# lucidrains/phenaki-pytorch

Measured on AMD Instinct MI355X. Metric: cvivit_encode_frames_per_sec, higher is better.
Workload: dtype bf16; 1 GPU; BASELINE configs[1]: C-ViViT (dim 512, patch 32, tpatch 2, depth 4+4, LFQ 65536) encode video -> token ids, (8,3,17,256,256) f32 per GPU resident in HBM; global_batch=8, parallelism=batch-shard x1, no data-path collective, hip_graph=True

## Files before the change

### include/phenaki_hip.h

```cpp
#ifndef PHENAKI_HIP_H
#define PHENAKI_HIP_H

#ifdef __cplusplus
extern "C" {
#endif

#define PK_OK 0
#define PK_EINVAL (-1)
#define PK_EALIGN (-2)
#define PK_ELAUNCH (-3)

int pk_gemm(int dtype, int a_is_f32, const void* A, int lda, const void* W, int ldw, int M, int N, int K,
            const float* bias, const float* res, int ldr, void* C, int ldc, int out_is_f32, int act,
            const int* a_rows, void* stream);

int pk_gemm_ex(int dtype, int a_is_f32, const void* A, int lda, const void* W, int ldw, int M, int N, int K,
               const float* bias, const float* res, int ldr, void* C, int ldc, int out_is_f32, int act,
               const int* a_rows, int a_nrows, int variant, void* C2, int ldc2, const float* ln_s, const float* ln_t,
               float ln_eps, const int* row_off, const int* col_off, float* stats_out, const float* ln_stats, int dup_rows,
               void* stream);
int pk_gemm_auto_variant(int dtype, int a_is_f32, int M, int N, int K, int lda, int ldw, int a_nrows);

int pk_layernorm(const float* x, int ldx, const float* gamma, const float* beta, float eps, void* out, int ldo,
                 int out_kind, float* out2, int ldo2, void* raw, int ldraw, int M, int D, int grp, int gstride,
// ... 46 lines not shown
int pk_lfq_aux_codebook(const float* Q, int cd, float inv_n, float coef, float* G, float* hc_part, void* stream);
int pk_lfq_aux_grad(const float* proj, const float* GA, const float* GB, int M, int cd, float alpha, float scale, float wen, float wc2,
                    float* dproj, void* stream);
int pk_lfq_aux_finish(const float* ent, const float* commit, int M, const float* hc_part, int cd, float w_e, float gamma, float w_c, float* out,
                      void* stream);

int pk_rmsnorm(const float* x, int ldx, const float* w, float eps, const unsigned char* rowmask, void* out, int ldo, int out_kind,
               int M, int D, void* stream);
int pk_gated_gelu_tanh(const float* h, int ldh, void* out, int ldo, int out_kind, int M, int F, void* stream);

int pk_layernorm_lfq(const float* x, int ldx, const float* gamma, const float* beta, float eps, const float* wp,
                     const float* bp, long long* ids, float* tokens, int ldt, float* proj, int M, int D, int cd,
                     int pb, int pc, void* stream);

int pk_l2norm_rows(const float* x, int ldx, void* out, int ldo, int out_kind, int M, int D, void* stream);

int pk_embed(const long long* ids_prime, int n_prime, const long long* ids, int n, int nb, const float* tok,
             const float* pos, float* out, void* out_t, int S, int D, void* stream);

int pk_cpb_input(const float* w0, const float* b0, float* out, int d0, int d1, int d2, int nd, int D, void* stream);

int pk_attn_pads(int nq, int n_kv, int nnull, int* nq_pad, int* nk_pad);
int pk_attn_prep(int dtype, const float* q, int ldq, const float* kv, int ldkv, const float* null_kv,
                 const float* q_scale, const float* k_scale, float scale, void* Qp, void* Kp, void* Vt,
                 int S, int h, int nq, int n_kv, int nnull, void* stream);

int pk_qkv_project(int dtype, const void* xq, const void* xkv, int ld, const void* wq, const void* wkv, int ldw, int S, int nseq,
                   int h, int K, const float* q_scale, const float* k_scale, float scale, void* Qp, void* Kp, void* Vt,
                   int nq_pad, int nk_pad, const float* q_ln_s, void* stream);

int pk_qkv_attn(int dtype, const void* xq, const void* xkv, int ld, const void* wq, const void* wkv, int ldw, int S, int n, int h, int K,
                const float* q_scale, const float* k_scale, float scale, const float* bias, long bias_hstride, int bias_ld,
                const float* slopes, int causal, void* O, int ldo, const float* q_ln_s, void* stream);

int pk_q_attn_cached(int dtype, const void* xq, int ld, const void* wq, int ldw, int S, int n, int h, int K, const float* q_scale, float scale,
                     const float* q_ln_s, const void* Kp, const void* Vt, int nk_pad, int n_kv, int nnull,
                     const unsigned char* kmask, void* O, int ldo, void* stream);

int pk_attn_fwd(int dtype, const void* Qp, const void* Kp, const void* Vt, const float* bias, long bias_hstride,
                int bias_ld, const unsigned char* kmask, const float* slopes, int causal, void* O, int ldo,
                int out_is_f32, int S, int h, int nq, int n_kv, int nnull, const float* bias_tab, int tab_len,
                const int* pos_code, int code_off, int tab_run4, float score_bound, void* stream);
int pk_attn_fwd_lse(int dtype, const void* Qp, const void* Kp, const void* Vt, const float* bias, long bias_hstride,
                    int bias_ld, const unsigned char* kmask, const float* slopes, int causal, void* O, int ldo,
                    int out_is_f32, int S, int h, int nq, int n_kv, int nnull, float* lse, void* stream);

int pk_attn_small(const float* q, int ldq, const float* kv, int ldkv, const float* q_scale, const float* k_scale,
                  float scale, const float* bias, long bias_hstride, int bias_ld, const unsigned char* kmask,
                  const float* slopes, int causal, void* O, int ldo, int out_kind, int S, int h, int n, void* stream);

int pk_cfg_mix(const float* x, int ldx, int nb, int n_tot, int n_prime, const int* rows, int nrows, float scale,
               int has_null, void* out, int ldo, int out_is_f32, int D, void* stream);

int pk_vocab_ntiles(int V);
int pk_vocab_sample(int dtype, const void* A, int lda, const void* W, int ldw, const float* bias, int M, int V, int D,
                    float temperature, const float* U, const int* rows, unsigned long long seed,
                    const unsigned long long* seed_dev, int need_lse, void* partials, void* stream);
int pk_vocab_sample_philox(int dtype, const void* A, int lda, const void* W, int ldw, const float* bias, int M, int V, int D, float temperature,
                           const int* rows, unsigned long long torch_seed, unsigned long long philox_offset, unsigned int philox_stride,
                           int need_lse, void* partials, void* stream);
int pk_vocab_reduce(const void* partials, int M, int V, const int* rows, const unsigned char* mask, long long* ids,
                    long long* pred, float* scores, int need_lse, void* stream);

int pk_vocab_ce(int dtype, const void* partials, int M, int V, const void* A, int lda, const void* W, int ldw,
                const float* bias, int D, const long long* targets, const int* rows, float* loss, float* lse_out, void* stream);
int pk_ce_grad_slab(int out_bf16, const float* logits, int ldl, const float* lse, const long long* targets, const int* rows,
// ... 77 lines not shown
```

### phenaki_pytorch_amd/_lib.py

```python
import ctypes
import os

import torch

_HERE = os.path.dirname(os.path.abspath(__file__))
LIB_PATH = os.environ.get('PK_LIB_PATH') or os.path.join(_HERE, 'libphenaki_hip.so')

_P = ctypes.c_void_p
_I = ctypes.c_int
_F = ctypes.c_float
_L = ctypes.c_long
_LL = ctypes.c_longlong
_ULL = ctypes.c_ulonglong

SIGNATURES = {
    'pk_gemm': [_I, _I, _P, _I, _P, _I, _I, _I, _I, _P, _P, _I, _P, _I, _I, _I, _P, _P],
    'pk_gemm_ex': [_I, _I, _P, _I, _P, _I, _I, _I, _I, _P, _P, _I, _P, _I, _I, _I, _P, _I, _I, _P, _I, _P, _P, _F, _P, _P, _P, _P, _I, _P],
    'pk_gemm_auto_variant': [_I, _I, _I, _I, _I, _I, _I, _I],
    'pk_layernorm': [_P, _I, _P, _P, _F, _P, _I, _I, _P, _I, _P, _I, _I, _I, _I, _I, _I, _I, _I, _P],
    'pk_rmsnorm': [_P, _I, _P, _F, _P, _P, _I, _I, _I, _I, _P],
    'pk_gated_gelu_tanh': [_P, _I, _P, _I, _I, _I, _I, _P],
    'pk_l2norm_rows': [_P, _I, _P, _I, _I, _I, _I, _P],
    'pk_patchify_ln': [_P, _I, _I, _I, _I, _I, _I, _I, _I, _I, _I, _P, _P, _F, _P, _I, _I, _P],
    'pk_patch_embed': [_P, _I, _I, _I, _I, _I, _I, _I, _I, _F, _I,
                       _P, _I, _P, _P, _P, _I, _I, _I,
                       _P, _I, _P, _P, _P, _I, _I, _I, _I, _P],
    'pk_patch_embed_slices': [_I],
    'pk_patch_embed_splitk': [_P, _I, _I, _I, _I, _I, _I, _I, _I, _I,
                              _P, _I, _P, _P, _I, _I, _I,
                              _P, _I, _P, _P, _I, _I, _I, _P],
    'pk_patch_embed_finish': [_P, _P, _I, _I, _I, _I, _P, _P, _F, _P, _P, _F, _P, _I, _P, _I, _I, _I, _I, _P],
    'pk_patch_embed_finish_groups': [_P, _I, _I, _P, _I, _P, _I, _P],
    'pk_patch_frame_mask': [_P, _LL, _P, _LL, _P, _I, _I, _I, _I, _I, _I, _I, _I, _I, _I, _P],
    'pk_unpatchify': [_P, _I, _P, _I, _I, _I, _I, _I, _I, _I, _I, _I, _I, _P],
    'pk_sqdiff_partials': [_P, _P, _P, _I, _I, _I, _I, _I, _P, _P],
    'pk_peg': [_P, _P, _P, _P, _P, _I, _I, _I, _I, _I, _I, _P],
    'pk_lfq_encode': [_P, _I, _P, _P, _P, _P, _I, _I, _I, _P],
    'pk_lfq_decode': [_P, _P, _P, _P, _I, _I, _I, _P, _I, _I, _I, _I, _P],
    'pk_lfq_aux_parts': [_I],
    'pk_lfq_aux_prep': [_P, _I, _I, _F, _F, _P, _P, _P, _P, _P],
    'pk_lfq_aux_codebook': [_P, _I, _F, _F, _P, _P, _P],
    'pk_lfq_aux_grad': [_P, _P, _P, _I, _I, _F, _F, _F, _F, _P, _P],
    'pk_lfq_aux_finish': [_P, _P, _I, _P, _I, _F, _F, _F, _P, _P],
    'pk_layernorm_lfq': [_P, _I, _P, _P, _F, _P, _P, _P, _P, _I, _P, _I, _I, _I, _I, _I, _P],
    'pk_embed': [_P, _I, _P, _I, _I, _P, _P, _P, _P, _I, _I, _P],
    'pk_cpb_input': [_P, _P, _P, _I, _I, _I, _I, _I, _P],
    'pk_attn_pads': [_I, _I, _I, ctypes.POINTER(_I), ctypes.POINTER(_I)],
    'pk_attn_prep': [_I, _P, _I, _P, _I, _P, _P, _P, _F, _P, _P, _P, _I, _I, _I, _I, _I, _P],
    'pk_qkv_project': [_I, _P, _P, _I, _P, _P, _I, _I, _I, _I, _I, _P, _P, _F, _P, _P, _P, _I, _I, _P, _P],
    'pk_qkv_attn': [_I, _P, _P, _I, _P, _P, _I, _I, _I, _I, _I, _P, _P, _F, _P, _L, _I, _P, _I, _P, _I, _P, _P],
    'pk_q_attn_cached': [_I, _P, _I, _P, _I, _I, _I, _I, _I, _P, _F, _P, _P, _P, _I, _I, _I, _P, _P, _I, _P],
    'pk_attn_fwd': [_I, _P, _P, _P, _P, _L, _I, _P, _P, _I, _P, _I, _I, _I, _I, _I, _I, _I, _P, _I, _P, _I, _I, _F, _P],
    'pk_attn_fwd_lse': [_I, _P, _P, _P, _P, _L, _I, _P, _P, _I, _P, _I, _I, _I, _I, _I, _I, _I, _P, _P],
    'pk_attn_small': [_P, _I, _P, _I, _P, _P, _F, _P, _L, _I, _P, _P, _I, _P, _I, _I, _I, _I, _I, _P],
    'pk_cfg_mix': [_P, _I, _I, _I, _I, _P, _I, _F, _I, _P, _I, _I, _I, _P],
    'pk_vocab_ntiles': [_I],
    'pk_vocab_sample_philox': [_I, _P, _I, _P, _I, _P, _I, _I, _I, _F, _P, _ULL, _ULL, ctypes.c_uint, _I, _P, _P],
    'pk_vocab_sample': [_I, _P, _I, _P, _I, _P, _I, _I, _I, _F, _P, _P, _ULL, _P, _I, _P, _P],
    'pk_vocab_reduce': [_P, _I, _I, _P, _P, _P, _P, _P, _I, _P],
    'pk_vocab_ce': [_I, _P, _I, _I, _P, _I, _P, _I, _P, _I, _P, _P, _P, _P, _P],
    'pk_ce_grad_slab': [_I, _P, _I, _P, _P, _P, _I, _I, _I, _F, _P, _P, _I, _P, _I, _P, _P],
    'pk_topk_mask': [_P, _I, _I, _I, _LL, _P, _P, _P, _P, _P],
    'pk_critic_head': [_P, _I, _P, _P, _I, _I, _I, _I, _I, _F, _P, _F, _ULL, _P, _P, _P],
    'pk_pack': [_P, _LL, _P, _I, _I, _I, _P, _LL, _I, _I, _P],
    'pk_scatter_rows': [_P, _LL, _P, _P, _LL, _I, _I, _P],
    'pk_colsum_parts': [_I],
    'pk_colsum': [_P, _LL, _I, _I, _F, _P, _I, _P, _P],
    'pk_ln_bwd_parts': [_I],
    'pk_layernorm_bwd': [_P, _LL, _P, _P, _LL, _P, _LL, _P, _LL, _P, _P, _F, _I, _I, _P],
    'pk_geglu': [_P, _LL, _I, _P, _LL, _I, _I, _P],
    'pk_geglu_bwd': [_P, _LL, _I, _P, _LL, _P, _LL, _I, _I, _P],
    'pk_leaky_bwd': [_P, _LL, _P, _LL, _P, _LL, _I, _I, _F, _P],
    'pk_scaled_diff': [_P, _P, _F, _P, _P, _LL, _P],
    'pk_sign': [_P, _F, _P, _LL, _P],
    'pk_mul': [_P, _P, _P, _LL, _P],
    'pk_peg_wgrad_parts': [_LL],
    'pk_peg_bwd': [_P, _P, _P, _P, _P, _I, _I, _I, _I, _I, _I, _P],
    'pk_embed_bwd': [_P, _P, _F, _P, _P, _I, _I, _I, _P],
    'pk_bias_gather': [_P, _I, _P, _I, _P, _I, _I, _P],
    'pk_bias_scatter': [_P, _P, _I, _P, _I, _I, _I, _P],
    'pk_sum_batch': [_P, _LL, _I, _P, _LL, _P],
    'pk_sum_batch_multi': [_P, _I, _P],
    'pk_peg_adjoint': [_P, _P, _P, _I, _I, _I, _I, _I, _I, _P],
# ... 278 lines not shown


def attn_prep(dtype, q, kv, null_kv, q_scale, k_scale, scale, Qp, Kp, Vt, S, h, nq, n_kv, nnull):
    rc = load().pk_attn_prep(dtype, ptr(q), q.stride(-2), ptr(kv), kv.stride(-2) if kv is not None else 0, f32p(null_kv, 'null_kv') if nnull else None,
                             f32p(q_scale, 'q_scale'), f32p(k_scale, 'k_scale'), scale, ptr(Qp), ptr(Kp), ptr(Vt), S, h, nq, n_kv, nnull, stream(q))
    _check(rc, 'pk_attn_prep')


def rmsnorm(x, w, M, D, out, eps=1e-6, rowmask=None):
    rc = load().pk_rmsnorm(f32p(x, 'x', rows_ok=True), x.stride(-2), f32p(w, 'T5LayerNorm weight'), eps, ptr(rowmask), ptr(out), out.stride(-2),
                           1 if out.dtype == torch.bfloat16 else 0, M, D, stream(x))
    _check(rc, 'pk_rmsnorm')


def gated_gelu_tanh(h, out, M, F):
    rc = load().pk_gated_gelu_tanh(ptr(h), h.stride(-2), ptr(out), out.stride(-2), 1 if out.dtype == torch.bfloat16 else 0, M, F, stream(h))
    _check(rc, 'pk_gated_gelu_tanh')


def _qkv_dtype(xq):
    if xq.dtype == torch.bfloat16:
        return BF16
    if xq.dtype == torch.float32:
        return BF16X3
    raise RuntimeError(f'fused projection kernels take bf16 (bf16 mode) or f32 (bf16x3 mode) rows, got {xq.dtype}')


def qkv_project(xq, xkv, wq, wkv, S, nseq, h, K, q_scale, k_scale, scale, Qp, Kp, Vt, nq_pad, nk_pad, q_ln_s=None):
    rc = load().pk_qkv_project(_qkv_dtype(xq), ptr(xq), ptr(xkv), xq.stride(-2), ptr(wq), ptr(wkv), wq.stride(0), S, nseq, h, K, f32p(q_scale, 'q_scale'),
                                f32p(k_scale, 'k_scale'), scale, ptr(Qp), ptr(Kp), ptr(Vt), nq_pad, nk_pad, ptr(q_ln_s), stream(xq))
    _check(rc, 'pk_qkv_project')


def qkv_attn(xq, xkv, wq, wkv, S, n, h, K, q_scale, k_scale, scale, O, *, bias=None, slopes=None, causal=False, q_ln_s=None):
    bh, bld = (bias.stride(0), bias.stride(1)) if bias is not None else (0, 0)
    rc = load().pk_qkv_attn(_qkv_dtype(xq), ptr(xq), ptr(xkv), xq.stride(-2), ptr(wq), ptr(wkv), wq.stride(0), S, n, h, K, f32p(q_scale, 'q_scale'),
                            f32p(k_scale, 'k_scale'), scale, f32p(bias, 'attention bias'), bh, bld, f32p(slopes, 'ALiBi slopes'),
                            1 if causal else 0, ptr(O), O.stride(-2), ptr(q_ln_s), stream(xq))
    _check(rc, 'pk_qkv_attn')


def q_attn_cached(xq, wq, S, n, h, K, q_scale, scale, Kp, Vt, nk_pad, n_kv, nnull, O, *, kmask=None, q_ln_s=None):
    rc = load().pk_q_attn_cached(_qkv_dtype(xq), ptr(xq), xq.stride(-2), ptr(wq), wq.stride(0), S, n, h, K, f32p(q_scale, 'q_scale'), scale, ptr(q_ln_s),
                                 ptr(Kp), ptr(Vt), nk_pad, n_kv, nnull, ptr(kmask), ptr(O), O.stride(-2), stream(xq))
    _check(rc, 'pk_q_attn_cached')


def attn_fwd(dtype, Qp, Kp, Vt, O, S, h, nq, n_kv, nnull, *, bias=None, kmask=None, slopes=None, causal=False, bias_table=None,
             score_bound=None, lse=None):
    tab, codes, off = bias_table[:3] if bias_table is not None else (None, None, 0)
    run4 = 1 if (bias_table is not None and len(bias_table) > 5 and bias_table[5]) else 0
    if bias is not None:
        bh, bld = bias.stride(0), bias.stride(1)
    else:
        bh, bld = 0, 0
    if lse is not None:
        assert bias_table is None and score_bound is None
        rc = load().pk_attn_fwd_lse(dtype, ptr(Qp), ptr(Kp), ptr(Vt), ptr(bias), bh, bld, ptr(kmask), f32p(slopes, 'ALiBi slopes'),
                                    1 if causal else 0, ptr(O), O.stride(-2), 1 if O.dtype == torch.float32 else 0, S, h, nq, n_kv, nnull, ptr(lse), stream(O))
        _check(rc, 'pk_attn_fwd_lse')
        return
    rc = load().pk_attn_fwd(dtype, ptr(Qp), ptr(Kp), ptr(Vt), ptr(bias), bh, bld, ptr(kmask), f32p(slopes, 'ALiBi slopes'),
                            1 if causal else 0, ptr(O), O.stride(-2), 1 if O.dtype == torch.float32 else 0,
                            S, h, nq, n_kv, nnull, f32p(tab, 'bias table'), tab.shape[1] if tab is not None else 0, ptr(codes), off, run4,
                            float('nan') if score_bound is None else float(score_bound), stream(O))
    _check(rc, 'pk_attn_fwd')


def attn_small(q, kv, q_scale, k_scale, scale, O, S, h, n, *, bias=None, kmask=None, slopes=None, causal=False):
    bh, bld = (bias.stride(0), bias.stride(1)) if bias is not None else (0, 0)
    rc = load().pk_attn_small(ptr(q), q.stride(-2), ptr(kv), kv.stride(-2), f32p(q_scale, 'q_scale'), f32p(k_scale, 'k_scale'), scale, ptr(bias), bh, bld,
                              ptr(kmask), f32p(slopes, 'ALiBi slopes'), 1 if causal else 0, ptr(O), O.stride(-2),
# ... 383 lines not shown
```

### phenaki_pytorch_amd/csrc/gemm_dma.hpp

```cpp
#pragma once
#include "gemm_core.hpp"

namespace pk {

__device__ __forceinline__ void dot2acc_bf16(float& d, uint32_t a, uint32_t b) {
    asm("v_dot2c_f32_bf16 %0, %1, %2" : "+v"(d) : "v"(a), "v"(b));
}
__device__ __forceinline__ void frag_stats(const Frag<bf16>& f, float& s, float& q, bool want_sq) {
    const uint32_t w0 = f.v[0], w1 = f.v[1], w2 = f.v[2], w3 = f.v[3];
    const uint32_t ones = 0x3f803f80u;
    dot2acc_bf16(s, w0, ones); dot2acc_bf16(s, w1, ones); dot2acc_bf16(s, w2, ones); dot2acc_bf16(s, w3, ones);
    if (want_sq) { dot2acc_bf16(q, w0, w0); dot2acc_bf16(q, w1, w1); dot2acc_bf16(q, w2, w2); dot2acc_bf16(q, w3, w3); }
}
__device__ __forceinline__ void frag_stats(const Frag<float>& f, float& s, float& q, bool want_sq) {
#pragma unroll
    for (int e = 0; e < 4; ++e) {
        s += f.lo[e] + f.hi[e];
        if (want_sq) q = fmaf(f.lo[e], f.lo[e], fmaf(f.hi[e], f.hi[e], q));
    }
}

#ifdef PK_TIMELINE
__device__ unsigned long long pk_tl[8 * 5 * 40];
#define PK_TL(slot) do { if (tl_on && kt < 38) pk_tl[(tl_wg * 40 + kt) * 5 + (slot)] = __builtin_amdgcn_s_memtime(); } while (0)
// ... 137 lines not shown
#pragma unroll
            for (int c = 0; c < CH; ++c) {
                Frag<T> fa[TM], fw[TN];
#pragma unroll
                for (int i = 0; i < TM; ++i) lds_frag_a<T>(fa[i], a, wm * 16 * TM + i * 16 + lr, c, g);
#pragma unroll
                for (int j = 0; j < TN; ++j) lds_frag_w<T>(fw[j], w, wn * 16 * TN + j * 16 + lr, c, g);
#pragma unroll
                for (int i = 0; i < TM; ++i)
#pragma unroll
                    for (int j = 0; j < TN; ++j) acc[i][j] = mma(fw[j], fa[i], acc[i][j]);
                if (STATS) {
#pragma unroll
                    for (int i = 0; i < TM; ++i) frag_stats(fa[i], rsum[i], rsq[i], STATS > 1);
                }
            }
            PK_TL(4);
        }
        if (STATS) {
#pragma unroll
            for (int i = 0; i < TM; ++i) {
                rsum[i] += __shfl_xor(rsum[i], 16, 64);
                rsum[i] += __shfl_xor(rsum[i], 32, 64);
                if (STATS > 1) {
                    rsq[i] += __shfl_xor(rsq[i], 16, 64);
                    rsq[i] += __shfl_xor(rsq[i], 32, 64);
                }
            }
        }
        asm volatile("s_waitcnt lgkmcnt(0)" ::: "memory");
        __builtin_amdgcn_s_barrier();
        return computes;
    }
};

}
```

### phenaki_pytorch_amd/csrc/qkv_attn.hip

```cpp
#include "gemm_dma.hpp"

namespace pk {

struct QkvAttnArgs {
    const void* xq; const void* xkv;
    const void* wq; const void* wkv;
    int ld, ldw;
    int S, n, h, K;
    int spt;
    const float* q_scale; const float* k_scale; float scale;
    const float* bias; long bias_hstride; int bias_ld;
    const float* slopes; int causal;
    void* O; int ldo;
    uint32_t recip;
    const float* q_ln_s;
};

template <typename T> using QaTile = GemmDma<T, 1, 4, 4, 1, 2, 128>;
template <typename T> using QaKvTile = GemmDma<T, 1, 8, 4, 1, 2, 128>;
constexpr int QA_SMEM = QaKvTile<bf16>::SMEM;
static_assert(QaKvTile<bf16x3>::SMEM == QA_SMEM, "the split-bf16 ring has the same bytes");

constexpr int QA_PLANE = 8192;
template <typename T> struct QaImg { static constexpr int PLANES = 1; };
template <> struct QaImg<bf16x3> { static constexpr int PLANES = 2; };
__device__ __forceinline__ void qa_put4(bf16, char* img, int off, f32x4 v) {
    *reinterpret_cast<u32x2*>(img + off) = u32x2{pack_bf2(v[0], v[1]), pack_bf2(v[2], v[3])};
}
__device__ __forceinline__ void qa_put4(bf16x3, char* img, int off, f32x4 v) {
    const uint32_t h0 = pack_bf2(v[0], v[1]), h1 = pack_bf2(v[2], v[3]);
    const float r0 = v[0] - __builtin_bit_cast(float, h0 << 16), r1 = v[1] - __builtin_bit_cast(float, h0 & 0xFFFF0000u);
    const float r2 = v[2] - __builtin_bit_cast(float, h1 << 16), r3 = v[3] - __builtin_bit_cast(float, h1 & 0xFFFF0000u);
    *reinterpret_cast<u32x2*>(img + off) = u32x2{h0, h1};
    *reinterpret_cast<u32x2*>(img + QA_PLANE + off) = u32x2{pack_bf2(r0, r1), pack_bf2(r2, r3)};
}
__device__ __forceinline__ void qa_put1(bf16, char* img, int off, float v) { *reinterpret_cast<u16*>(img + off) = f2bf(v); }
__device__ __forceinline__ void qa_put1(bf16x3, char* img, int off, float v) {
    const u16 h = f2bf(v);
    *reinterpret_cast<u16*>(img + off) = h;
    *reinterpret_cast<u16*>(img + QA_PLANE + off) = f2bf(v - bf2f(h));
}
__device__ __forceinline__ void qa_get(Frag<bf16>& f, const char* img, int off) { f.v = *reinterpret_cast<const u32x4*>(img + off); }
__device__ __forceinline__ void qa_get(Frag<bf16x3>& f, const char* img, int off) {
    f.hi = *reinterpret_cast<const u32x4*>(img + off);
    f.lo = *reinterpret_cast<const u32x4*>(img + QA_PLANE + off);
}

__device__ __forceinline__ int qa_kperm(int f, int i) { return (f >> 1) * 32 + (i >> 2) * 8 + (f & 1) * 4 + (i & 3); }
__device__ __forceinline__ int qa_ksw(int row) { return ((row >> 1) & 1) | (((row >> 3) & 3) << 1); }

template <typename T>
__device__ __forceinline__ void qa_project_q(const GemmOperands& p, int M, int m0, int hh, int K, const float* q_scale, float scale,
                                             const float* q_ln_s, char* smem, char* Qs) {
    const int lane = threadIdx.x & 63, g = lane >> 4, lr = lane & 15;
    const int rq = __builtin_amdgcn_readfirstlane(threadIdx.x >> 6) * 16 + lr;
    f32x4 acc[1][4];
#pragma unroll
    for (int j = 0; j < 4; ++j) acc[0][j] = f32x4{0, 0, 0, 0};
    if (q_ln_s) {
        float rsum[1], rsq[1];
        (void)QaTile<T>::template run_stats<1>(p, M, m0, hh * 64, smem, acc, rsum, rsq);
        const float mean = rsum[0] / (float)K;
#pragma unroll
        for (int j = 0; j < 4; ++j) {
            const f32x4 s4 = *reinterpret_cast<const f32x4*>(q_ln_s + hh * 64 + j * 16 + g * 4);
#pragma unroll
            for (int r = 0; r < 4; ++r) acc[0][j][r] -= mean * s4[r];
        }
    } else {
        (void)QaTile<T>::run(p, M, m0, hh * 64, smem, acc);
    }
    float ss = 0.f;
#pragma unroll
    for (int j = 0; j < 4; ++j)
#pragma unroll
        for (int r = 0; r < 4; ++r) ss += acc[0][j][r] * acc[0][j][r];
    ss += __shfl_xor(ss, 16, 64);
    ss += __shfl_xor(ss, 32, 64);
    const float inv = scale / fmaxf(sqrtf(ss), 1e-12f);
#pragma unroll
    for (int j = 0; j < 4; ++j) {
        const f32x4 sc = *reinterpret_cast<const f32x4*>(q_scale + j * 16 + g * 4);
        f32x4 v = acc[0][j];
#pragma unroll
        for (int r = 0; r < 4; ++r) v[r] *= inv * sc[r];
        const int slot = (2 * j + (g >> 1)) ^ (rq & 7);
        qa_put4(T{}, Qs, rq * 128 + (slot << 4) + (g & 1) * 8, v);
    }
}

template <typename T>
__global__ __launch_bounds__(256) void qkv_attn_kernel(const QkvAttnArgs a) {
    extern __shared__ __attribute__((aligned(16))) char smem[];
    constexpr int NPL = QaImg<T>::PLANES;
    char* Qs = smem;
    char* Ks = smem;
    char* Vts = smem + NPL * QA_PLANE;
    const int R = a.spt * a.n;
    const int tiles = (a.S + a.spt - 1) / a.spt;
    const int xcd = blockIdx.x & 7, idx = blockIdx.x >> 3;
    const int tile = (idx / a.h) * 8 + xcd, hh = idx % a.h;
    if (tile >= tiles) return;
    const int M = a.S * a.n;
    const int m0 = tile * R;
    const int lane = threadIdx.x & 63, g = lane >> 4, lr = lane & 15;
    const int wave = __builtin_amdgcn_readfirstlane(threadIdx.x >> 6);
    const int rq = wave * 16 + lr;

    GemmOperands p;
    p.a_rows = nullptr;
    p.lda = a.ld; p.ldw = a.ldw;
    p.M = M; p.K = a.K;
    p.plain_map = 0; p.krot = 0;
    p.w_gap_from = 0; p.w_gap_rows = 0;

    p.A = a.xq; p.W = a.wq; p.N = a.h * 64;
    qa_project_q<T>(p, M, m0, hh, a.K, a.q_scale, a.scale, a.q_ln_s, smem, Qs);
    Frag<T> fq[2];
    asm volatile("s_waitcnt lgkmcnt(0)" ::: "memory");
#pragma unroll
    for (int c = 0; c < 2; ++c) qa_get(fq[c], Qs, rq * 128 + (((c * 4 + g) ^ (rq & 7)) << 4));
    asm volatile("s_waitcnt lgkmcnt(0)" ::: "memory");
    __builtin_amdgcn_s_barrier();

    {
        f32x4 acc[1][8];
#pragma unroll
        for (int j = 0; j < 8; ++j) acc[0][j] = f32x4{0, 0, 0, 0};
        p.A = a.xkv; p.W = a.wkv; p.N = 2 * a.h * 64;
        p.w_gap_from = 64; p.w_gap_rows = (a.h - 1) * 64;
        (void)QaKvTile<T>::run(p, M, m0, hh * 64, smem, acc);
        float ss = 0.f;
#pragma unroll
        for (int j = 0; j < 4; ++j)
#pragma unroll
            for (int r = 0; r < 4; ++r) ss += acc[0][j][r] * acc[0][j][r];
        ss += __shfl_xor(ss, 16, 64);
        ss += __shfl_xor(ss, 32, 64);
        const float inv = 1.0f / fmaxf(sqrtf(ss), 1e-12f);
#pragma unroll
        for (int j = 0; j < 4; ++j) {
            const f32x4 sc = *reinterpret_cast<const f32x4*>(a.k_scale + j * 16 + g * 4);
            f32x4 v = acc[0][j];
#pragma unroll
            for (int r = 0; r < 4; ++r) v[r] *= inv * sc[r];
            const int slot = (2 * j + (g >> 1)) ^ qa_ksw(rq);
            qa_put4(T{}, Ks, rq * 128 + (slot << 4) + (g & 1) * 8, v);
        }
#pragma unroll
        for (int j = 0; j < 4; ++j)
#pragma unroll
            for (int r = 0; r < 4; ++r) {
                const int d = j * 16 + g * 4 + r;
                qa_put1(T{}, Vts, d * 128 + ((((rq >> 3) ^ (d & 7))) << 4) + (rq & 7) * 2, acc[0][4 + j][r]);
            }
    }
    asm volatile("s_waitcnt lgkmcnt(0)" ::: "memory");
    __builtin_amdgcn_s_barrier();

    f32x4 st[4];
#pragma unroll
    for (int f = 0; f < 4; ++f) st[f] = f32x4{0, 0, 0, 0};
#pragma unroll
    for (int f = 0; f < 4; ++f) {
// ... 179 lines not shown
    mx = fmaxf(mx, __shfl_xor(mx, 32, 64));
    float ls = 0.f;
#pragma unroll
    for (int e = 0; e < 4 * NF; ++e) { pr[e] = __expf(pr[e] - mx); ls += pr[e]; }
    ls += __shfl_xor(ls, 16, 64);
    ls += __shfl_xor(ls, 32, 64);
    f32x4 o[4];
#pragma unroll
    for (int df = 0; df < 4; ++df) o[df] = f32x4{0, 0, 0, 0};
#pragma unroll
    for (int kc = 0; kc < NF / 2; ++kc) {
        Frag<T> fp;
        {
            const float p8[8] = {pr[kc * 8 + 0], pr[kc * 8 + 1], pr[kc * 8 + 2], pr[kc * 8 + 3], pr[kc * 8 + 4], pr[kc * 8 + 5], pr[kc * 8 + 6], pr[kc * 8 + 7]};
            frag_from_f32(fp, p8);
        }
#pragma unroll
        for (int df = 0; df < 4; ++df) {
            const int d = df * 16 + lr;
            Frag<T> fv;
            qa_get(fv, Vts, d * 128 + (((kc * 4 + g) ^ (d & 7)) << 4));
            o[df] = mma(fv, fp, o[df]);
        }
    }
    const float inv = 1.0f / ls;
    T* orow = reinterpret_cast<T*>(a.O) + (size_t)(m0 + rq) * a.ldo + hh * 64;
#pragma unroll
    for (int df = 0; df < 4; ++df) store4(orow + df * 16 + g * 4, o[df] * inv);
}

}
using namespace pk;

extern "C" int pk_qkv_attn(int dtype, const void* xq, const void* xkv, int ld, const void* wq, const void* wkv, int ldw, int S, int n, int h,
                           int K, const float* q_scale, const float* k_scale, float scale, const float* bias, long bias_hstride,
                           int bias_ld, const float* slopes, int causal, void* O, int ldo, const float* q_ln_s, void* stream) {
    if (dtype != 1 && dtype != 2) return PK_EINVAL;
    if (!xq || !xkv || !wq || !wkv || !q_scale || !k_scale || !O || S <= 0 || n <= 0 || n > 64 || h <= 0 || K <= 0) return PK_EINVAL;
    auto mis = [](const void* ptr) { return (reinterpret_cast<uintptr_t>(ptr) & 15) != 0; };
    const int q = dtype == 1 ? 7 : 3, bk = dtype == 1 ? 64 : 32, esz = dtype == 1 ? 2 : 4;
    if ((K & q) || (ld & q) || (ldw & q) || (ldo & 3) || mis(xq) || mis(xkv) || mis(wq) || mis(wkv) || mis(q_scale) || mis(k_scale) ||
        (reinterpret_cast<uintptr_t>(O) & (dtype == 1 ? 7 : 15)) || (bias && mis(bias))) return PK_EALIGN;
    if (ldw < (K + bk - 1) / bk * bk) return PK_EINVAL;
    const long M = (long)S * n;
    if ((size_t)M * ld * esz >= 0xFFFFFFF0ull || (size_t)2 * h * 64 * ldw * esz >= 0xFFFFFFF0ull) return PK_EINVAL;
    QkvAttnArgs a;
    a.xq = xq; a.xkv = xkv; a.wq = wq; a.wkv = wkv; a.ld = ld; a.ldw = ldw;
    a.S = S; a.n = n; a.h = h; a.K = K; a.spt = 64 / n;
    a.q_scale = q_scale; a.k_scale = k_scale; a.scale = scale;
    a.bias = bias; a.bias_hstride = bias_hstride; a.bias_ld = bias_ld;
    a.slopes = slopes; a.causal = causal;
    a.O = O; a.ldo = ldo;
    a.recip = (65536u + (uint32_t)n - 1u) / (uint32_t)n;
    a.q_ln_s = q_ln_s;
    if (q_ln_s && mis(q_ln_s)) return PK_EALIGN;
    const int tiles = (S + a.spt - 1) / a.spt;
    dim3 grid(8 * ((tiles + 7) / 8) * h);
    hipStream_t st = reinterpret_cast<hipStream_t>(stream);
    if (dtype == 1) hipLaunchKernelGGL(qkv_attn_kernel<bf16>, grid, dim3(256), QA_SMEM, st, a);
    else hipLaunchKernelGGL(qkv_attn_kernel<bf16x3>, grid, dim3(256), QA_SMEM, st, a);
    PK_CHECK_LAUNCH();
    return PK_OK;
}

extern "C" int pk_q_attn_cached(int dtype, const void* xq, int ld, const void* wq, int ldw, int S, int n, int h, int K, const float* q_scale,
                                float scale, const float* q_ln_s, const void* Kp, const void* Vt, int nk_pad, int n_kv, int nnull,
                                const unsigned char* kmask, void* O, int ldo, void* stream) {
    if (dtype != 1 && dtype != 2) return PK_EINVAL;
    if (!xq || !wq || !q_scale || !Kp || !Vt || !O || S <= 0 || n <= 0 || (n & 63) || h <= 0 || K <= 0 || n_kv <= 0 || nnull < 0) return PK_EINVAL;
    const int nk = nnull + n_kv;
    if (nk > 64 || nk_pad < nk || nk_pad > 64 || (nk_pad & 31)) return PK_EINVAL;
    auto mis = [](const void* ptr) { return (reinterpret_cast<uintptr_t>(ptr) & 15) != 0; };
    const int q = dtype == 1 ? 7 : 3, bk = dtype == 1 ? 64 : 32, esz = dtype == 1 ? 2 : 4;
    if ((K & q) || (ld & q) || (ldw & q) || (ldo & 3) || mis(xq) || mis(wq) || mis(q_scale) || mis(Kp) || mis(Vt) ||
        (reinterpret_cast<uintptr_t>(O) & (dtype == 1 ? 7 : 15)) || (q_ln_s && mis(q_ln_s))) return PK_EALIGN;
    if (dtype == 2 && ((reinterpret_cast<uintptr_t>(Kp) | reinterpret_cast<uintptr_t>(Vt)) & 127)) return PK_EALIGN;
    if (ldw < (K + bk - 1) / bk * bk) return PK_EINVAL;
    const long M = (long)S * n;
    if ((size_t)M * ld * esz >= 0xFFFFFFF0ull || (size_t)h * 64 * ldw * esz >= 0xFFFFFFF0ull) return PK_EINVAL;
    QAttnCachedArgs a{xq, wq, ld, ldw, S, n, h, K, q_scale, scale, q_ln_s, Kp, Vt, nk_pad, nk, nnull, kmask, n_kv, O, ldo};
    const int tiles = (int)(M / 64);
    dim3 grid(8 * ((tiles + 7) / 8) * h);
    hipStream_t st = reinterpret_cast<hipStream_t>(stream);
    if (dtype == 1) {
        constexpr int lds = QaTile<bf16>::SMEM + 2 * QA_PLANE;
        if (nk_pad > 32) hipLaunchKernelGGL((q_attn_cached_kernel<bf16, true>), grid, dim3(256), lds, st, a);
        else hipLaunchKernelGGL((q_attn_cached_kernel<bf16, false>), grid, dim3(256), lds, st, a);
    } else {
        constexpr int lds = QaTile<bf16x3>::SMEM + 4 * QA_PLANE;
        if (nk_pad > 32) hipLaunchKernelGGL((q_attn_cached_kernel<bf16x3, true>), grid, dim3(256), lds, st, a);
        else hipLaunchKernelGGL((q_attn_cached_kernel<bf16x3, false>), grid, dim3(256), lds, st, a);
    }
    PK_CHECK_LAUNCH();
    return PK_OK;
}
// ... 1 lines not shown
```

Before: 177,200 frames/s.

## Overlap K/V projection prefetch with Q projection tail in fused qkv-attention kernel

```diff
diff --git a/include/phenaki_hip.h b/include/phenaki_hip.h
--- a/include/phenaki_hip.h
+++ b/include/phenaki_hip.h
@@ -102,6 +102,9 @@
 int pk_qkv_attn(int dtype, const void* xq, const void* xkv, int ld, const void* wq, const void* wkv, int ldw, int S, int n, int h, int K,
                 const float* q_scale, const float* k_scale, float scale, const float* bias, long bias_hstride, int bias_ld,
                 const float* slopes, int causal, void* O, int ldo, const float* q_ln_s, void* stream);
+int pk_qkv_attn_ex(int dtype, const void* xq, const void* xkv, int ld, const void* wq, const void* wkv, int ldw, int S, int n, int h, int K,
+                   const float* q_scale, const float* k_scale, float scale, const float* bias, long bias_hstride, int bias_ld,
+                   const float* slopes, int causal, void* O, int ldo, const float* q_ln_s, int sched, void* stream);
 
 int pk_q_attn_cached(int dtype, const void* xq, int ld, const void* wq, int ldw, int S, int n, int h, int K, const float* q_scale, float scale,
                      const float* q_ln_s, const void* Kp, const void* Vt, int nk_pad, int n_kv, int nnull,
diff --git a/phenaki_pytorch_amd/_lib.py b/phenaki_pytorch_amd/_lib.py
--- a/phenaki_pytorch_amd/_lib.py
+++ b/phenaki_pytorch_amd/_lib.py
@@ -49,6 +49,7 @@
     'pk_attn_prep': [_I, _P, _I, _P, _I, _P, _P, _P, _F, _P, _P, _P, _I, _I, _I, _I, _I, _P],
     'pk_qkv_project': [_I, _P, _P, _I, _P, _P, _I, _I, _I, _I, _I, _P, _P, _F, _P, _P, _P, _I, _I, _P, _P],
     'pk_qkv_attn': [_I, _P, _P, _I, _P, _P, _I, _I, _I, _I, _I, _P, _P, _F, _P, _L, _I, _P, _I, _P, _I, _P, _P],
+    'pk_qkv_attn_ex': [_I, _P, _P, _I, _P, _P, _I, _I, _I, _I, _I, _P, _P, _F, _P, _L, _I, _P, _I, _P, _I, _P, _I, _P],
     'pk_q_attn_cached': [_I, _P, _I, _P, _I, _I, _I, _I, _I, _P, _F, _P, _P, _P, _I, _I, _I, _P, _P, _I, _P],
     'pk_attn_fwd': [_I, _P, _P, _P, _P, _L, _I, _P, _P, _I, _P, _I, _I, _I, _I, _I, _I, _I, _P, _I, _P, _I, _I, _F, _P],
     'pk_attn_fwd_lse': [_I, _P, _P, _P, _P, _L, _I, _P, _P, _I, _P, _I, _I, _I, _I, _I, _I, _I, _P, _P],
@@ -393,12 +394,15 @@
     _check(rc, 'pk_qkv_project')
 
 
-def qkv_attn(xq, xkv, wq, wkv, S, n, h, K, q_scale, k_scale, scale, O, *, bias=None, slopes=None, causal=False, q_ln_s=None):
+QKV_ATTN_PIPE = 0 if os.environ.get('PK_QKV_ATTN_PIPE', '1') == '0' else 1
+
+
+def qkv_attn(xq, xkv, wq, wkv, S, n, h, K, q_scale, k_scale, scale, O, *, bias=None, slopes=None, causal=False, q_ln_s=None, sched=None):
     bh, bld = (bias.stride(0), bias.stride(1)) if bias is not None else (0, 0)
-    rc = load().pk_qkv_attn(_qkv_dtype(xq), ptr(xq), ptr(xkv), xq.stride(-2), ptr(wq), ptr(wkv), wq.stride(0), S, n, h, K, f32p(q_scale, 'q_scale'),
-                            f32p(k_scale, 'k_scale'), scale, f32p(bias, 'attention bias'), bh, bld, f32p(slopes, 'ALiBi slopes'),
-                            1 if causal else 0, ptr(O), O.stride(-2), ptr(q_ln_s), stream(xq))
-    _check(rc, 'pk_qkv_attn')
+    rc = load().pk_qkv_attn_ex(_qkv_dtype(xq), ptr(xq), ptr(xkv), xq.stride(-2), ptr(wq), ptr(wkv), wq.stride(0), S, n, h, K, f32p(q_scale, 'q_scale'),
+                               f32p(k_scale, 'k_scale'), scale, f32p(bias, 'attention bias'), bh, bld, f32p(slopes, 'ALiBi slopes'),
+                               1 if causal else 0, ptr(O), O.stride(-2), ptr(q_ln_s), QKV_ATTN_PIPE if sched is None else sched, stream(xq))
+    _check(rc, 'pk_qkv_attn_ex')
 
 
 def q_attn_cached(xq, wq, S, n, h, K, q_scale, scale, Kp, Vt, nk_pad, n_kv, nnull, O, *, kmask=None, q_ln_s=None):
diff --git a/phenaki_pytorch_amd/csrc/gemm_dma.hpp b/phenaki_pytorch_amd/csrc/gemm_dma.hpp
--- a/phenaki_pytorch_amd/csrc/gemm_dma.hpp
+++ b/phenaki_pytorch_amd/csrc/gemm_dma.hpp
@@ -193,6 +193,130 @@
         __builtin_amdgcn_s_barrier();
         return computes;
     }
+
+    struct Feed {
+        __amdgpu_buffer_rsrc_t rsA, rsW;
+        uint32_t offA[IA], offW[IW], bytesA;
+        int wave, nt, rot;
+        bool slot_in_tail;
+
+        __device__ __forceinline__ Feed(const GemmOperands& p, int a_nrows, int m0, int n0, int wave_) : wave(wave_) {
+            constexpr int SZ = (int)sizeof(T);
+            const int lane = threadIdx.x & 63;
+            bytesA = (uint32_t)a_nrows * (uint32_t)p.lda * SZ;
+            const uint32_t bytesW = (uint32_t)p.N * (uint32_t)p.ldw * SZ;
+            rsA = __builtin_amdgcn_make_buffer_rsrc(const_cast<void*>(p.A), 0, bytesA, 0x00020000);
+            rsW = __builtin_amdgcn_make_buffer_rsrc(const_cast<void*>(p.W), 0, bytesW, 0x00020000);
+            const int lrow = lane / SLOTS, lslot = lane % SLOTS;
+            const int srcslot = lslot ^ (lrow & 7);
+#pragma unroll
+            for (int i = 0; i < IA; ++i) {
+                const int row = (wave * IA + i) * RPI + lrow;
+                int gm = m0 + row;
+                const bool ok = gm < p.M;
+                if (ok && p.a_rows) gm = p.a_rows[gm];
+                offA[i] = ok ? (uint32_t)gm * (uint32_t)p.lda * SZ + srcslot * 16 : bytesA;
+            }
+#pragma unroll
+            for (int i = 0; i < IW; ++i) {
+                const int row = (wave * IW + i) * RPI + lrow;
+                const int gn = n0 + row + ((p.w_gap_from > 0 && row >= p.w_gap_from) ? p.w_gap_rows : 0);
+                offW[i] = gn < p.N ? (uint32_t)gn * (uint32_t)p.ldw * SZ + srcslot * 16 : bytesW;
+            }
+            nt = (p.K + BK - 1) / BK;
+            rot = (p.krot && nt > 1) ? (int)(((blockIdx.x >> 3) + blockIdx.y) % (unsigned)nt) : 0;
+            const int ktail_bytes = (p.K * SZ) % ROWB;
+            slot_in_tail = ktail_bytes == 0 || srcslot * 16 < ktail_bytes;
+        }
+
+        __device__ __forceinline__ void issue(int kt, char* base) const {
+            int kk = kt + rot;
+            if (kk >= nt) kk -= nt;
+            const int koff = kk * ROWB;
+            const bool cut = kk == nt - 1 && !slot_in_tail;
+#pragma unroll
+            for (int i = 0; i < IA; ++i)
+                __builtin_amdgcn_raw_ptr_buffer_load_lds(rsA, (lds_ptr)(base + (wave * IA + i) * 1024), 16, cut ? bytesA : offA[i], koff, 0, 0);
+#pragma unroll
+            for (int i = 0; i < IW; ++i)
+                __builtin_amdgcn_raw_ptr_buffer_load_lds(rsW, (lds_ptr)(base + BM * ROWB + (wave * IW + i) * 1024), 16, offW[i], koff, 0, 0);
+        }
+    };
+
+    template <int STATS>
+    static __device__ __forceinline__ void mma_tile(const char* a, int wm, int wn, int lr, int g, f32x4 (&acc)[TM][TN], float (&rsum)[TM],
+                                                    float (&rsq)[TM]) {
+        const char* w = a + BM * ROWB;
+#pragma unroll
+        for (int c = 0; c < CH; ++c) {
+            Frag<T> fa[TM], fw[TN];
+#pragma unroll
+            for (int i = 0; i < TM; ++i) lds_frag_a<T>(fa[i], a, wm * 16 * TM + i * 16 + lr, c, g);
+#pragma unroll
+            for (int j = 0; j < TN; ++j) lds_frag_w<T>(fw[j], w, wn * 16 * TN + j * 16 + lr, c, g);
+#pragma unroll
+            for (int i = 0; i < TM; ++i)
+#pragma unroll
+                for (int j = 0; j < TN; ++j) acc[i][j] = mma(fw[j], fa[i], acc[i][j]);
+            if (STATS) {
+#pragma unroll
+                for (int i = 0; i < TM; ++i) frag_stats(fa[i], rsum[i], rsq[i], STATS > 1);
+            }
+        }
+    }
+
+    template <int STATS>
+    static __device__ __forceinline__ void fold_stats(float (&rsum)[TM], float (&rsq)[TM]) {
+        if (STATS) {
+#pragma unroll
+            for (int i = 0; i < TM; ++i) {
+                rsum[i] += __shfl_xor(rsum[i], 16, 64);
+                rsum[i] += __shfl_xor(rsum[i], 32, 64);
+                if (STATS > 1) {
+                    rsq[i] += __shfl_xor(rsq[i], 16, 64);
+                    rsq[i] += __shfl_xor(rsq[i], 32, 64);
+                }
+            }
+        }
+    }
+
+    template <int STATS, bool ISSUED0, bool CLOSE, typename Seam>
+    static __device__ __forceinline__ void chain(const Feed& feed, char* st0, char* st1, f32x4 (&acc)[TM][TN], float (&rsum)[TM],
+                                                 float (&rsq)[TM], Seam seam) {
+        static_assert(STAGES == 2 && PW == 0, "chained passes: 2-stage ring, no producer waves");
+        const int lane = threadIdx.x & 63, g = lane >> 4, lr = lane & 15;
+        const int cw = feed.wave, wm = cw / WN, wn = cw % WN;
+        const int nt = feed.nt;
+        if (STATS) {
+#pragma unroll
+            for (int i = 0; i < TM; ++i) { rsum[i] = 0.f; rsq[i] = 0.f; }
+        }
+        if (!ISSUED0) feed.issue(0, st0);
+        for (int kt = 0; kt < nt - 1; ++kt) {
+            wait_tiles<0>();
+            __builtin_amdgcn_s_barrier();
+            feed.issue(kt + 1, (kt + 1) & 1 ? st1 : st0);
+            mma_tile<STATS>(kt & 1 ? st1 : st0, wm, wn, lr, g, acc, rsum, rsq);
+        }
+        wait_tiles<0>();
+        __builtin_amdgcn_s_barrier();
+        seam();
+        mma_tile<STATS>((nt - 1) & 1 ? st1 : st0, wm, wn, lr, g, acc, rsum, rsq);
+        fold_stats<STATS>(rsum, rsq);
+        if (CLOSE) {
+            asm volatile("s_waitcnt lgkmcnt(0)" ::: "memory");
+            __builtin_amdgcn_s_barrier();
+        }
+    }
+    template <int STATS, typename Seam>
+    static __device__ __forceinline__ void run_lead(const Feed& feed, char* st0, char* st1, f32x4 (&acc)[TM][TN], float (&rsum)[TM],
+                                                    float (&rsq)[TM], Seam seam) {
+        chain<STATS, false, false>(feed, st0, st1, acc, rsum, rsq, seam);
+    }
+    static __device__ __forceinline__ void run_issued(const Feed& feed, char* st0, char* st1, f32x4 (&acc)[TM][TN]) {
+        float dummy[TM];
+        chain<0, true, true>(feed, st0, st1, acc, dummy, dummy, [] {});
+    }
 };
 
 }
diff --git a/phenaki_pytorch_amd/csrc/qkv_attn.hip b/phenaki_pytorch_amd/csrc/qkv_attn.hip
--- a/phenaki_pytorch_amd/csrc/qkv_attn.hip
+++ b/phenaki_pytorch_amd/csrc/qkv_attn.hip
@@ -50,6 +50,38 @@
 __device__ __forceinline__ int qa_ksw(int row) { return ((row >> 1) & 1) | (((row >> 3) & 3) << 1); }
 
 template <typename T>
+__device__ __forceinline__ void qa_finish_q(f32x4 (&acc)[1][4], bool has_ln, float rsum, int K, const f32x4 (&ln4)[4], const f32x4 (&qs4)[4],
+                                            float scale, char* Qs, int rq, int g) {
+    if (has_ln) {
+        const float mean = rsum / (float)K;
+#pragma unroll
+        for (int j = 0; j < 4; ++j)
+#pragma unroll
+            for (int r = 0; r < 4; ++r) acc[0][j][r] -= mean * ln4[j][r];
+    }
+    float ss = 0.f;
+#pragma unroll
+    for (int j = 0; j < 4; ++j)
+#pragma unroll
+        for (int r = 0; r < 4; ++r) ss += acc[0][j][r] * acc[0][j][r];
+    ss += __shfl_xor(ss, 16, 64);
+    ss += __shfl_xor(ss, 32, 64);
+    const float inv = scale / fmaxf(sqrtf(ss), 1e-12f);
+#pragma unroll
+    for (int j = 0; j < 4; ++j) {
+        f32x4 v = acc[0][j];
+#pragma unroll
+        for (int r = 0; r < 4; ++r) v[r] *= inv * qs4[j][r];
+        const int slot = (2 * j + (g >> 1)) ^ (rq & 7);
+        qa_put4(T{}, Qs, rq * 128 + (slot << 4) + (g & 1) * 8, v);
+    }
+}
+__device__ __forceinline__ void qa_load_cols(f32x4 (&v)[4], const float* base, int g) {
+#pragma unroll
+    for (int j = 0; j < 4; ++j) v[j] = *reinterpret_cast<const f32x4*>(base + j * 16 + g * 4);
+}
+
+template <typename T>
 __device__ __forceinline__ void qa_project_q(const GemmOperands& p, int M, int m0, int hh, int K, const float* q_scale, float scale,
                                              const float* q_ln_s, char* smem, char* Qs) {
     const int lane = threadIdx.x & 63, g = lane >> 4, lr = lane & 15;
@@ -57,40 +89,21 @@
     f32x4 acc[1][4];
 #pragma unroll
     for (int j = 0; j < 4; ++j) acc[0][j] = f32x4{0, 0, 0, 0};
+    float rsum[1] = {0.f}, rsq[1];
+    f32x4 ln4[4], qs4[4];
     if (q_ln_s) {
-        float rsum[1], rsq[1];
         (void)QaTile<T>::template run_stats<1>(p, M, m0, hh * 64, smem, acc, rsum, rsq);
-        const float mean = rsum[0] / (float)K;
-#pragma unroll
-        for (int j = 0; j < 4; ++j) {
-            const f32x4 s4 = *reinterpret_cast<const f32x4*>(q_ln_s + hh * 64 + j * 16 + g * 4);
-#pragma unroll
-            for (int r = 0; r < 4; ++r) acc[0][j][r] -= mean * s4[r];
-        }
+        qa_load_cols(ln4, q_ln_s + hh * 64, g);
     } else {
         (void)QaTile<T>::run(p, M, m0, hh * 64, smem, acc);
     }
-    float ss = 0.f;
-#pragma unroll
-    for (int j = 0; j < 4; ++j)
-#pragma unroll
-        for (int r = 0; r < 4; ++r) ss += acc[0][j][r] * acc[0][j][r];
-    ss += __shfl_xor(ss, 16, 64);
-    ss += __shfl_xor(ss, 32, 64);
-    const float inv = scale / fmaxf(sqrtf(ss), 1e-12f);
-#pragma unroll
-    for (int j = 0; j < 4; ++j) {
-        const f32x4 sc = *reinterpret_cast<const f32x4*>(q_scale + j * 16 + g * 4);
-        f32x4 v = acc[0][j];
-#pragma unroll
-        for (int r = 0; r < 4; ++r) v[r] *= inv * sc[r];
-        const int slot = (2 * j + (g >> 1)) ^ (rq & 7);
-        qa_put4(T{}, Qs, rq * 128 + (slot << 4) + (g & 1) * 8, v);
-    }
-}
-
-template <typename T>
+    qa_load_cols(qs4, q_scale, g);
+    qa_finish_q<T>(acc, q_ln_s != nullptr, rsum[0], K, ln4, qs4, scale, Qs, rq, g);
+}
+
+template <typename T, bool PIPE>
 __global__ __launch_bounds__(256) void qkv_attn_kernel(const QkvAttnArgs a) {
+    static_assert(!PIPE || QaImg<T>::PLANES == 1, "the seam-free schedule stages ONE 8 KB q^ plane beside the k|v stage being filled");
     extern __shared__ __attribute__((aligned(16))) char smem[];
     constexpr int NPL = QaImg<T>::PLANES;
     char* Qs = smem;
@@ -114,22 +127,55 @@
     p.plain_map = 0; p.krot = 0;
     p.w_gap_from = 0; p.w_gap_rows = 0;
 
-    p.A = a.xq; p.W = a.wq; p.N = a.h * 64;
-    qa_project_q<T>(p, M, m0, hh, a.K, a.q_scale, a.scale, a.q_ln_s, smem, Qs);
     Frag<T> fq[2];
-    asm volatile("s_waitcnt lgkmcnt(0)" ::: "memory");
-#pragma unroll
-    for (int c = 0; c < 2; ++c) qa_get(fq[c], Qs, rq * 128 + (((c * 4 + g) ^ (rq & 7)) << 4));
-    asm volatile("s_waitcnt lgkmcnt(0)" ::: "memory");
-    __builtin_amdgcn_s_barrier();
-
-    {
-        f32x4 acc[1][8];
-#pragma unroll
-        for (int j = 0; j < 8; ++j) acc[0][j] = f32x4{0, 0, 0, 0};
+    f32x4 acc[1][8];
+#pragma unroll
+    for (int j = 0; j < 8; ++j) acc[0][j] = f32x4{0, 0, 0, 0};
+    if constexpr (PIPE) {
+        using QT = QaTile<T>;
+        using KT = QaKvTile<T>;
+        const int nt = (a.K + QT::BK - 1) / QT::BK;
+        const int s0 = nt & 1;
+        char* const kv0 = smem + s0 * KT::STAGE_BYTES;
+        char* const kv1 = smem + (s0 ^ 1) * KT::STAGE_BYTES;
+        Qs = smem + (s0 ? 2 : 3) * QA_PLANE;
+        p.A = a.xq; p.W = a.wq; p.N = a.h * 64;
+        const typename QT::Feed feed_q(p, M, m0, hh * 64, wave);
+        p.A = a.xkv; p.W = a.wkv; p.N = 2 * a.h * 64;
+        p.w_gap_from = 64; p.w_gap_rows = (a.h - 1) * 64;
+        const typename KT::Feed feed_kv(p, M, m0, hh * 64, wave);
+        f32x4 qacc[1][4];
+#pragma unroll
+        for (int j = 0; j < 4; ++j) qacc[0][j] = f32x4{0, 0, 0, 0};
+        float rsum[1] = {0.f}, rsq[1];
+        f32x4 ln4[4], qs4[4];
+        auto seam = [&] {
+            if (a.q_ln_s) qa_load_cols(ln4, a.q_ln_s + hh * 64, g);
+            qa_load_cols(qs4, a.q_scale, g);
+            asm volatile("" ::: "memory");
+            feed_kv.issue(0, kv0);
+        };
+        if (a.q_ln_s) QT::template run_lead<1>(feed_q, smem, smem + 4 * QA_PLANE, qacc, rsum, rsq, seam);
+        else QT::template run_lead<0>(feed_q, smem, smem + 4 * QA_PLANE, qacc, rsum, rsq, seam);
+        qa_finish_q<T>(qacc, a.q_ln_s != nullptr, rsum[0], a.K, ln4, qs4, a.scale, Qs, rq, g);
+        asm volatile("s_waitcnt lgkmcnt(0)" ::: "memory");
+#pragma unroll
+        for (int c = 0; c < 2; ++c) qa_get(fq[c], Qs, rq * 128 + (((c * 4 + g) ^ (rq & 7)) << 4));
+        asm volatile("s_waitcnt lgkmcnt(0)" ::: "memory");
+        KT::run_issued(feed_kv, kv0, kv1, acc);
+    } else {
+        p.A = a.xq; p.W = a.wq; p.N = a.h * 64;
+        qa_project_q<T>(p, M, m0, hh, a.K, a.q_scale, a.scale, a.q_ln_s, smem, Qs);
+        asm volatile("s_waitcnt lgkmcnt(0)" ::: "memory");
+#pragma unroll
+        for (int c = 0; c < 2; ++c) qa_get(fq[c], Qs, rq * 128 + (((c * 4 + g) ^ (rq & 7)) << 4));
+        asm volatile("s_waitcnt lgkmcnt(0)" ::: "memory");
+        __builtin_amdgcn_s_barrier();
         p.A = a.xkv; p.W = a.wkv; p.N = 2 * a.h * 64;
         p.w_gap_from = 64; p.w_gap_rows = (a.h - 1) * 64;
         (void)QaKvTile<T>::run(p, M, m0, hh * 64, smem, acc);
+    }
+    {
         float ss = 0.f;
 #pragma unroll
         for (int j = 0; j < 4; ++j)
@@ -375,10 +421,11 @@
 }
 using namespace pk;
 
-extern "C" int pk_qkv_attn(int dtype, const void* xq, const void* xkv, int ld, const void* wq, const void* wkv, int ldw, int S, int n, int h,
-                           int K, const float* q_scale, const float* k_scale, float scale, const float* bias, long bias_hstride,
-                           int bias_ld, const float* slopes, int causal, void* O, int ldo, const float* q_ln_s, void* stream) {
+extern "C" int pk_qkv_attn_ex(int dtype, const void* xq, const void* xkv, int ld, const void* wq, const void* wkv, int ldw, int S, int n, int h,
+                              int K, const float* q_scale, const float* k_scale, float scale, const float* bias, long bias_hstride,
+                              int bias_ld, const float* slopes, int causal, void* O, int ldo, const float* q_ln_s, int sched, void* stream) {
     if (dtype != 1 && dtype != 2) return PK_EINVAL;
+    if (sched != 0 && sched != 1) return PK_EINVAL;
     if (!xq || !xkv || !wq || !wkv || !q_scale || !k_scale || !O || S <= 0 || n <= 0 || n > 64 || h <= 0 || K <= 0) return PK_EINVAL;
     auto mis = [](const void* ptr) { return (reinterpret_cast<uintptr_t>(ptr) & 15) != 0; };
     const int q = dtype == 1 ? 7 : 3, bk = dtype == 1 ? 64 : 32, esz = dtype == 1 ? 2 : 4;
@@ -400,10 +447,18 @@
     const int tiles = (S + a.spt - 1) / a.spt;
     dim3 grid(8 * ((tiles + 7) / 8) * h);
     hipStream_t st = reinterpret_cast<hipStream_t>(stream);
-    if (dtype == 1) hipLaunchKernelGGL(qkv_attn_kernel<bf16>, grid, dim3(256), QA_SMEM, st, a);
-    else hipLaunchKernelGGL(qkv_attn_kernel<bf16x3>, grid, dim3(256), QA_SMEM, st, a);
+    if (dtype == 1 && sched == 1) hipLaunchKernelGGL((qkv_attn_kernel<bf16, true>), grid, dim3(256), QA_SMEM, st, a);
+    else if (dtype == 1) hipLaunchKernelGGL((qkv_attn_kernel<bf16, false>), grid, dim3(256), QA_SMEM, st, a);
+    else hipLaunchKernelGGL((qkv_attn_kernel<bf16x3, false>), grid, dim3(256), QA_SMEM, st, a);
     PK_CHECK_LAUNCH();
     return PK_OK;
+}
+
+extern "C" int pk_qkv_attn(int dtype, const void* xq, const void* xkv, int ld, const void* wq, const void* wkv, int ldw, int S, int n, int h,
+                           int K, const float* q_scale, const float* k_scale, float scale, const float* bias, long bias_hstride,
+                           int bias_ld, const float* slopes, int causal, void* O, int ldo, const float* q_ln_s, void* stream) {
+    return pk_qkv_attn_ex(dtype, xq, xkv, ld, wq, wkv, ldw, S, n, h, K, q_scale, k_scale, scale, bias, bias_hstride, bias_ld, slopes, causal, O, ldo,
+                          q_ln_s, 1, stream);
 }
 
 extern "C" int pk_q_attn_cached(int dtype, const void* xq, int ld, const void* wq, int ldw, int S, int n, int h, int K, const float* q_scale,
```

After: 177,200 frames/s, median of 3. About the same (+0.0%).
